# YikangZhang1641/merging-gym

Measured on AMD Instinct MI355X. Metric: env-steps/sec at batch=2^20; achieved HBM GB/s vs peak; 1/2/4/8-GPU scaling, higher is better.
Workload: dtype f64

## Files before the change

### merging-gym_amd/csrc/mg_qnet.h

```cpp
#pragma once

#include "mg_common.h"

namespace {

typedef __bf16 bf16x8 __attribute__((ext_vector_type(8)));
typedef float f32x16 __attribute__((ext_vector_type(16)));
typedef short i16x2 __attribute__((ext_vector_type(2)));
typedef __bf16 bf16x2 __attribute__((ext_vector_type(2)));

constexpr int kQH1Real = 200, kQH2Real = 100;
constexpr int kQT1 = 7;
constexpr int kQT2 = 7;
constexpr int kQK3 = 4;
constexpr int kQBiasIn = 13;
constexpr int kQOne1 = 200;
constexpr int kQOne2 = 100;
constexpr int kQMaxIn = kQBiasIn;
constexpr int kLMaxOut = 8;
static_assert(32 * kQT1 >= kQOne1 + 3 && 32 * (kQT1 - 1) < kQH1Real && 16 * kQT2 >= kQOne2 + 3 &&
                  16 * (kQT2 - 1) < kQH2Real && 32 * kQK3 >= 16 * kQT2,
              "tile counts cover the hidden units and their 1.0 units, no tile is all padding");

struct QFrag {
  int kind, tile, kb;
};
constexpr int kQFrags = 1 + 6 * 8 + 11;
__host__ __device__ constexpr QFrag qfrag(int s) {
  if (s == 0) return QFrag{0, 0, 0};
  if (s < 49) {
    const int u = s - 1, kb = u / 8, v = u % 8;
    return v == 0 ? QFrag{0, kb + 1, 0} : QFrag{1, v - 1, kb};
  }
  const int u = s - 49;
  if (u == 10) return QFrag{2, 0, 3};
  return u % 3 == 0 && u > 0 ? QFrag{2, 0, u / 3 - 1} : QFrag{1, u - u / 3, kQT1 - 1};
}
__host__ __device__ constexpr int qfrag_off(int s) {
  if (s <= 49) return 1024 * s;
  const int u = s - 49;
  return 1024 * s - 512 * ((u > 3) + (u > 6) + (u > 9) + (u > 10));
}
constexpr int kQNetBytes = qfrag_off(kQFrags);
static_assert(kQNetBytes == 56 * 1024 + 4 * 512, "7 W1 + 49 W2 fragments of 1 KB, 4 W3 of 512 B");

__host__ __device__ constexpr int qnet_unit1(int kb, int g, int j) {
  return 32 * kb + (j & 3) + 8 * (j >> 2) + 16 * (g & 1) + 4 * (g >> 1);
}
__host__ __device__ constexpr int qnet_unit2(int kb, int g, int j) {
  return 32 * kb + 16 * (j >> 2) + 4 * g + (j & 3);
}

__device__ __forceinline__ uint32_t relu_pair(float x, float y) {
  i16x2 v = __builtin_bit_cast(i16x2, __builtin_convertvector(f32x2{x, y}, bf16x2));
  const i16x2 zero = {0, 0};
  v = __builtin_elementwise_max(v, zero);
  return __builtin_bit_cast(uint32_t, v);
}

__device__ __forceinline__ bf16x8 qnet_input(const float* row, bool swap, int h) {
  float v[kObs];
#pragma unroll
  for (int k = 0; k < kObs / 2; ++k) {
    const f32x2 t = reinterpret_cast<const f32x2*>(row)[k];
    v[2 * k] = t[0];
    v[2 * k + 1] = t[1];
  }
  uint32_t pr[kObs / 2];
#pragma unroll
  for (int k = 0; k < kObs / 2; ++k) {
    const int a = swap ? (2 * k + 5) % kObs : 2 * k, b = swap ? (2 * k + 6) % kObs : 2 * k + 1;
    pr[k] = __builtin_bit_cast(uint32_t, __builtin_convertvector(f32x2{v[a], v[b]}, bf16x2));
  }
  static_assert(kQBiasIn == 13 && kObs == 10, "bias slots 13..15 follow the 10 features");
  const u32x4 w = h ? u32x4{pr[4], 0u, 0x3F800000u, 0x3F803F80u} : u32x4{pr[0], pr[1], pr[2], pr[3]};
  return __builtin_bit_cast(bf16x8, w);
}

__device__ __forceinline__ bf16x8 qnet_input_wide(const float* row16, int h) {
  const f32x4 lo = reinterpret_cast<const f32x4*>(row16 + 8 * h)[0];
  const f32x4 hi = reinterpret_cast<const f32x4*>(row16 + 8 * h)[1];
  const u32x4 w = {__builtin_bit_cast(uint32_t, __builtin_convertvector(f32x2{lo[0], lo[1]}, bf16x2)),
                   __builtin_bit_cast(uint32_t, __builtin_convertvector(f32x2{lo[2], lo[3]}, bf16x2)),
                   __builtin_bit_cast(uint32_t, __builtin_convertvector(f32x2{hi[0], hi[1]}, bf16x2)),
                   __builtin_bit_cast(uint32_t, __builtin_convertvector(f32x2{hi[2], hi[3]}, bf16x2))};
  return __builtin_bit_cast(bf16x8, w);
}

__device__ __forceinline__ f32x16 mfma32(bf16x8 a, bf16x8 b, f32x16 c) {
  return __builtin_amdgcn_mfma_f32_32x32x16_bf16(a, b, c, 0, 0, 0);
}
__device__ __forceinline__ f32x4 mfma16(bf16x8 a, bf16x8 b, f32x4 c) {
  return __builtin_amdgcn_mfma_f32_16x16x32_bf16(a, b, c, 0, 0, 0);
}

__global__ void qnet_pack_kernel(const float* w1, const float* b1, const float* w2, const float* b2,
                                 const float* w3, const float* b3, int in_dim, int out_dim,
                                 uint8_t* packed) {
  const int e = blockIdx.x * blockDim.x + threadIdx.x;
  if (e >= kQFrags * 64 * 8) return;
  const int s = e >> 9, lane = (e >> 3) & 63, j = e & 7;
  const QFrag f = qfrag(s);
  auto part = [](float b, int p) {
    const float hi = static_cast<float>(static_cast<__bf16>(b));
    const float r = b - hi;
    const float mid = static_cast<float>(static_cast<__bf16>(r));
    return p == 0 ? hi : p == 1 ? mid : r - mid;
  };
  float v = 0.f;
  int off = qfrag_off(s) + 16 * lane;
  if (f.kind == 0) {
    const int m = 32 * f.tile + (lane & 31), k = 8 * (lane >> 5) + j;
    if (m < kQH1Real && k < in_dim) v = w1[m * in_dim + k];
    else if (m < kQH1Real && k >= kQBiasIn && k < kQBiasIn + 3) v = part(b1[m], k - kQBiasIn);
    else if (m >= kQOne1 && m < kQOne1 + 3 && k == kQBiasIn) v = 1.f;
  } else if (f.kind == 1) {
    const int m = 16 * f.tile + (lane & 15), u = qnet_unit1(f.kb, lane >> 4, j);
    if (m < kQH2Real && u < kQH1Real) v = w2[m * kQH1Real + u];
    else if (m < kQH2Real && u >= kQOne1 && u < kQOne1 + 3) v = part(b2[m], u - kQOne1);
    else if (m >= kQOne2 && m < kQOne2 + 3 && u == kQOne1) v = 1.f;
  } else {
    if ((lane & 15) >= 8) return;
    const int m = lane & 7, u = qnet_unit2(f.kb, lane >> 4, j);
    if (m < out_dim && u < kQH2Real) v = w3[m * kQH2Real + u];
    else if (m < out_dim && u >= kQOne2 && u < kQOne2 + 3) v = part(b3[m], u - kQOne2);
    off = qfrag_off(s) + 16 * (8 * (lane >> 4) + m);
  }
  reinterpret_cast<__bf16*>(packed + off)[j] = static_cast<__bf16>(v);
}

__device__ __forceinline__ int opaque_zero() {
  int z = 0;
  asm volatile("" : "+v"(z));
  return z;
}

__device__ __forceinline__ void qnet_to_lds(const uint8_t* net, uint8_t* lds) {
  const f32x4* src = reinterpret_cast<const f32x4*>(net);
  f32x4* dst = reinterpret_cast<f32x4*>(lds);
  for (int j = threadIdx.x; j < kQNetBytes / 16; j += blockDim.x) dst[j] = src[j];
}

struct QSrcLds {
  const uint8_t* net;
  int lo, lo3;
  __device__ __forceinline__ bf16x8 operator()(int s) const {
    return *reinterpret_cast<const bf16x8*>(net + qfrag_off(s) + (qfrag(s).kind == 2 ? lo3 : lo));
  }
};
struct QSrcGlobal {
  __amdgpu_buffer_rsrc_t rs;
  int lo, lo3;
  __device__ __forceinline__ bf16x8 operator()(int s) const {
    return __builtin_bit_cast(
        bf16x8, __builtin_amdgcn_raw_buffer_load_b128(rs, qfrag(s).kind == 2 ? lo3 : lo, qfrag_off(s), 0));
  }
};
__device__ __forceinline__ int qnet_lane_off() { return 16 * (threadIdx.x & 63); }
__device__ __forceinline__ int qnet_lane_off3() {
  const int lane = threadIdx.x & 63;
  return 16 * (8 * (lane >> 4) + (lane & 7));
}
__device__ __forceinline__ QSrcLds qnet_lds(const uint8_t* net) {
  return QSrcLds{net + opaque_zero(), qnet_lane_off(), qnet_lane_off3()};
}
__device__ __forceinline__ QSrcGlobal qnet_global(const uint8_t* net) {
  return QSrcGlobal{__builtin_amdgcn_make_buffer_rsrc(const_cast<uint8_t*>(net), static_cast<short>(0), kQNetBytes,
                                                      0x00020000),
                    qnet_lane_off(), qnet_lane_off3()};
}
constexpr int kQLdsAhead = 2;
constexpr int kQGlobalAhead = 3;

__device__ __forceinline__ void permlane16_swap(uint32_t& x, uint32_t& y) {
  const uint32_t a = x, b = y;
  const uint64_t sw = __builtin_bit_cast(uint64_t, __builtin_amdgcn_permlane16_swap(a, b, false, false));
  x = static_cast<uint32_t>(sw);
  y = static_cast<uint32_t>(sw >> 32);
}

__device__ __forceinline__ void qnet_gather_q(const f32x4 (&acc3)[4], float (&q)[8]) {
  float x0[4], y0[4], x1[4], y1[4];
#pragma unroll
  for (int i = 0; i < 4; ++i) {
    x0[i] = acc3[0][i];
    y0[i] = acc3[2][i];
    x1[i] = acc3[1][i];
    y1[i] = acc3[3][i];
  }
  asm volatile(
      "s_nop 7\n\ts_nop 7\n\t"
      "v_permlane32_swap_b32 %0, %4\n\tv_permlane32_swap_b32 %8, %12\n\t"
      "v_permlane32_swap_b32 %1, %5\n\tv_permlane32_swap_b32 %9, %13\n\t"
      "v_permlane32_swap_b32 %2, %6\n\tv_permlane32_swap_b32 %10, %14\n\t"
      "v_permlane32_swap_b32 %3, %7\n\tv_permlane32_swap_b32 %11, %15\n\t"
      "s_nop 1\n\t"
      "v_permlane16_swap_b32 %0, %8\n\tv_permlane16_swap_b32 %1, %9\n\t"
      "v_permlane16_swap_b32 %2, %10\n\tv_permlane16_swap_b32 %3, %11\n\t"
      "s_nop 1"
      : "+v"(x0[0]), "+v"(x0[1]), "+v"(x0[2]), "+v"(x0[3]), "+v"(y0[0]), "+v"(y0[1]), "+v"(y0[2]), "+v"(y0[3]),
        "+v"(x1[0]), "+v"(x1[1]), "+v"(x1[2]), "+v"(x1[3]), "+v"(y1[0]), "+v"(y1[1]), "+v"(y1[2]), "+v"(y1[3]));
#pragma unroll
  for (int i = 0; i < 4; ++i) {
    q[i] = x0[i];
    q[4 + i] = x1[i];
  }
}

template <int D, int NC = 4, class Src>
__device__ __forceinline__ void qnet_mlp(const Src& src, bf16x8 xb0, bf16x8 xb1, float (&q)[8]) {
  static_assert(NC >= 1 && NC <= 4, "1..4 column tiles");
  constexpr int nc = NC;
  static_assert(kQT1 == 7 && kQT2 == 7 && kQK3 == 4 && kQFrags == 60,
                "qfrag's consumption order assumes 7 k-blocks, 7 layer-2 row tiles and 4 layer-3 k-blocks");
  bf16x8 ring[D];
#pragma unroll
  for (int s = 0; s < D; ++s) ring[s] = src(s);
  auto take = [&](int s) __attribute__((always_inline)) {
    const bf16x8 f = ring[s % D];
    if (s + D < kQFrags) ring[s % D] = src(s + D);
    return f;
  };
  const f32x16 z16 = {};
  const f32x4 z4 = {};
  f32x16 c0, c1;
  constexpr bool hi = nc > 2;
  auto layer1 = [&](int s) __attribute__((always_inline)) {
    const bf16x8 a1 = take(s);
    c0 = mfma32(a1, xb0, z16);
    if (hi) c1 = mfma32(a1, xb1, z16);
  };
  auto relu_d = [&](int d) __attribute__((always_inline)) {
    const f32x16& c = d < 8 ? c0 : c1;
    const int b = 2 * (d & 7);
    return relu_pair(c[b], c[b + 1]);
  };
  uint32_t nx[16];
  auto swap_u = [&](int u) __attribute__((always_inline)) {
#pragma unroll
    for (int qd = 0; qd < 4; ++qd) permlane16_swap(nx[8 * u + qd], nx[8 * u + 4 + qd]);
  };
  auto operands = [&](bf16x8 (&hb)[4]) __attribute__((always_inline)) {
#pragma unroll
    for (int t = 0; t < 4; ++t) hb[t] = __builtin_bit_cast(bf16x8, u32x4{nx[4 * t], nx[4 * t + 1], nx[4 * t + 2], nx[4 * t + 3]});
  };
  layer1(0);
#pragma unroll
  for (int d = 0; d < 8; ++d) nx[d] = relu_d(d);
  if (hi) {
#pragma unroll
    for (int d = 8; d < 16; ++d) nx[d] = relu_d(d);
  }
  swap_u(0);
  if (hi) swap_u(1);
  bf16x8 hb[4];
  operands(hb);
  f32x4 acc2[kQT2][4];
  auto slot = [&](f32x4& acc, const bf16x8& a, const bf16x8& b, bool zero) __attribute__((always_inline)) {
    __builtin_amdgcn_sched_barrier(0);
    acc = mfma16(a, b, zero ? z4 : acc);
  };
  int s = 1;
#pragma unroll
  for (int kb = 0; kb < kQT1 - 1; ++kb) {
    layer1(s++);
#pragma unroll
    for (int t2 = 0; t2 < kQT2; ++t2) {
      const bf16x8 a2 = take(s++);
#pragma unroll
      for (int t = 0; t < 4; ++t) {
        if (t < nc) slot(acc2[t2][t], a2, hb[t], kb == 0);
        if (t2 >= 1 && t2 <= 4 && (t2 <= 2 || hi)) nx[4 * (t2 - 1) + t] = relu_d(4 * (t2 - 1) + t);
        if (t2 == 5) permlane16_swap(nx[t], nx[4 + t]);
        if (t2 == 6 && hi) permlane16_swap(nx[8 + t], nx[12 + t]);
      }
    }
    operands(hb);
  }
  f32x4 acc3[4] = {z4, z4, z4, z4};
  uint32_t b3[2][4][4];
  auto pairs3 = [&](int t2, int t) __attribute__((always_inline)) {
    const int buf = (t2 >> 1) & 1, d = 2 * (t2 & 1);
    b3[buf][t][d] = relu_pair(acc2[t2][t][0], acc2[t2][t][1]);
    b3[buf][t][d + 1] = relu_pair(acc2[t2][t][2], acc2[t2][t][3]);
  };
  auto layer2 = [&](int t2, int p) __attribute__((always_inline)) {
    const bf16x8 a2 = take(s++);
#pragma unroll
    for (int t = 0; t < 4; ++t) {
      if (t < nc) slot(acc2[t2][t], a2, hb[t], false);
      if (p >= 0 && t < nc) pairs3(p, t);
    }
  };
  auto layer3 = [&](int k3, int p) __attribute__((always_inline)) {
    const bf16x8 a3 = take(s++);
    const int buf = k3 & 1;
#pragma unroll
    for (int t = 0; t < 4; ++t) {
      if (2 * k3 + 1 >= kQT2) b3[buf][t][2] = b3[buf][t][3] = 0u;
      const bf16x8 b = __builtin_bit_cast(bf16x8, u32x4{b3[buf][t][0], b3[buf][t][1], b3[buf][t][2], b3[buf][t][3]});
      if (t < nc) slot(acc3[t], a3, b, k3 == 0);
      if (p >= 0 && t < nc) pairs3(p, t);
    }
  };
  static_assert(kQT2 == 7 && kQK3 == 4, "the tail below is written for 7 row tiles, 4 layer-3 k-blocks");
  layer2(0, -1);
  layer2(1, 0);
  layer2(2, 1);
  layer3(0, 2);
  layer2(3, -1);
  layer2(4, 3);
  layer3(1, 4);
  layer2(5, -1);
  layer2(6, 5);
  layer3(2, 6);
  layer3(3, -1);
  qnet_gather_q(acc3, q);
}

template <int D, class Src>
__device__ __forceinline__ void qnet_mlp_nc(const Src& src, bf16x8 xb0, bf16x8 xb1, float (&q)[8], int nc) {
  switch (nc) {
    case 1:
      qnet_mlp<4 * D, 1>(src, xb0, xb1, q);
      break;
    case 2:
      qnet_mlp<2 * D, 2>(src, xb0, xb1, q);
      break;
    case 3:
      qnet_mlp<D + D / 2, 3>(src, xb0, xb1, q);
      break;
    default:
      qnet_mlp<D, 4>(src, xb0, xb1, q);
  }
}

__device__ __forceinline__ void qnet_mlp_swp(const uint8_t* net, bf16x8 xb0, bf16x8 xb1, float (&q)[8]) {
  qnet_mlp<kQLdsAhead>(qnet_lds(net), xb0, xb1, q);
}
__device__ __forceinline__ void qnet_mlp_swp_nc(const uint8_t* net, bf16x8 xb0, bf16x8 xb1, float (&q)[8], int nc) {
  qnet_mlp_nc<kQLdsAhead>(qnet_lds(net), xb0, xb1, q, nc);
}

__device__ __forceinline__ void qnet_forward_swp(const uint8_t* net, const float* tile, int row0,
                                                 bool swap, float (&q)[8]) {
  const int lane = threadIdx.x & 63, r = lane & 31, h = lane >> 5;
  qnet_mlp_swp(net, qnet_input(tile + (row0 + r) * kObs, swap, h),
               qnet_input(tile + (row0 + 32 + r) * kObs, swap, h), q);
}

constexpr int kQ32H1 = 224, kQ32H2 = 128;
constexpr int kQ32S1 = 24, kQ32S2 = 232, kQ32S3 = 136;
constexpr int kQ32R1 = 204, kQ32R2 = 104, kQ32R3 = 9;
constexpr int kQ32OffW2 = kQ32R1 * kQ32S1 * 2;
constexpr int kQ32OffW3 = kQ32OffW2 + kQ32R2 * kQ32S2 * 2;
constexpr int kQ32NetBytes = kQ32OffW3 + kQ32R3 * kQ32S3 * 2;
static_assert(kQ32OffW2 % 16 == 0 && kQ32OffW3 % 16 == 0 && kQ32NetBytes % 16 == 0 && kQNetBytes % 16 == 0,
              "packed Q-net sections must stay 16-byte aligned");

__device__ __forceinline__ int q32row1(int m) { return m < kQ32R1 ? m : kQ32R1 - 1; }
__device__ __forceinline__ int q32row2(int m) { return m < kQ32R2 ? m : kQ32R2 - 1; }
__device__ __forceinline__ int q32row3(int m) { return m < kQ32R3 ? m : kQ32R3 - 1; }

__host__ __device__ constexpr int q32_krow(int kk) {
  return 8 * ((kk & 7) >> 2) + 4 * (kk >> 3) + (kk & 3);
}

__device__ __forceinline__ bf16x8 relu_bf16(const f32x16& c, int s) {
  const int b = 8 * s;
  return __builtin_bit_cast(bf16x8, u32x4{relu_pair(c[b], c[b + 1]), relu_pair(c[b + 2], c[b + 3]),
                                          relu_pair(c[b + 4], c[b + 5]), relu_pair(c[b + 6], c[b + 7])});
}

__global__ void qnet32_pack_kernel(const float* w1, const float* b1, const float* w2, const float* b2,
                                 const float* w3, const float* b3, int in_dim, int out_dim,
                                 uint8_t* packed) {
  int e = blockIdx.x * blockDim.x + threadIdx.x;
  __bf16* pw1 = reinterpret_cast<__bf16*>(packed);
  __bf16* pw2 = reinterpret_cast<__bf16*>(packed + kQ32OffW2);
  __bf16* pw3 = reinterpret_cast<__bf16*>(packed + kQ32OffW3);
  auto part = [](float b, int p) {
    const float hi = static_cast<float>(static_cast<__bf16>(b));
    const float r = b - hi;
    const float mid = static_cast<float>(static_cast<__bf16>(r));
    return p == 0 ? hi : p == 1 ? mid : r - mid;
  };
  if (e < kQ32R1 * kQ32S1) {
    const int m = e / kQ32S1, k = e % kQ32S1;
    float v = 0.f;
    if (m < kQH1Real && k < in_dim) v = w1[m * in_dim + k];
    else if (m < kQH1Real && k >= kQBiasIn && k < kQBiasIn + 3) v = part(b1[m], k - kQBiasIn);
    else if (m >= kQOne1 && m < kQOne1 + 3 && k == kQBiasIn) v = 1.f;
    pw1[e] = static_cast<__bf16>(v);
    return;
  }
  e -= kQ32R1 * kQ32S1;
  if (e < kQ32R2 * kQ32S2) {
    const int m = e / kQ32S2, c = e % kQ32S2;
    const int src = 16 * (c / 16) + q32_krow(c % 16);
    float v = 0.f;
    if (c < kQ32H1) {
      if (m < kQH2Real && src < kQH1Real) v = w2[m * kQH1Real + src];
      else if (m < kQH2Real && src >= kQOne1 && src < kQOne1 + 3) v = part(b2[m], src - kQOne1);
      else if (m >= kQOne2 && m < kQOne2 + 3 && src == kQOne1) v = 1.f;
    }
    pw2[e] = static_cast<__bf16>(v);
    return;
  }
  e -= kQ32R2 * kQ32S2;
  if (e < kQ32R3 * kQ32S3) {
    const int m = e / kQ32S3, c = e % kQ32S3;
    const int src = 16 * (c / 16) + q32_krow(c % 16);
    float v = 0.f;
    if (m < out_dim && c < kQ32H2) {
      if (src < kQH2Real) v = w3[m * kQH2Real + src];
      else if (src >= kQOne2 && src < kQOne2 + 3) v = part(b3[m], src - kQOne2);
    }
    pw3[e] = static_cast<__bf16>(v);
  }
}

__device__ __forceinline__ void qnet32_gather_q(const f32x16& acc3_0, const f32x16& acc3_1, int h,
                                              float (&q)[8]) {
  (void)h;
#pragma unroll
  for (int j = 0; j < 4; ++j) {
    const float a = acc3_0[j], b = acc3_1[j];
    const uint32_t x = __builtin_bit_cast(uint32_t, a), y = __builtin_bit_cast(uint32_t, b);
    const uint64_t sw = __builtin_bit_cast(uint64_t, __builtin_amdgcn_permlane32_swap(x, y, false, false));
    q[j] = __builtin_bit_cast(float, static_cast<uint32_t>(sw));
    q[4 + j] = __builtin_bit_cast(float, static_cast<uint32_t>(sw >> 32));
  }
}

__device__ __forceinline__ void qnet32_mlp(const uint8_t* net, bf16x8 xb0, bf16x8 xb1, float (&q)[8]) {
  const int lane = threadIdx.x & 63, r = lane & 31, h = lane >> 5;
  const int z = opaque_zero();
  const __bf16* W1 = reinterpret_cast<const __bf16*>(net) + z;
  const __bf16* W2 = reinterpret_cast<const __bf16*>(net + kQ32OffW2) + z;
  const __bf16* W3 = reinterpret_cast<const __bf16*>(net + kQ32OffW3) + z;
  f32x16 acc2a[4] = {}, acc2b[4] = {};
  const f32x16 zero = {};
  auto layer1 = [&](int mt, f32x16& c0, f32x16& c1) {
    const bf16x8 a1 = *reinterpret_cast<const bf16x8*>(W1 + q32row1(32 * mt + r) * kQ32S1 + 8 * h);
    c0 = mfma32(a1, xb0, zero);
    c1 = mfma32(a1, xb1, zero);
  };
  f32x16 c0, c1;
  layer1(0, c0, c1);
  bf16x8 hb[4] = {relu_bf16(c0, 0), relu_bf16(c0, 1), relu_bf16(c1, 0), relu_bf16(c1, 1)};
  auto w2frag = [&](int mt, int j) {
    return *reinterpret_cast<const bf16x8*>(W2 + q32row2(32 * (j >> 1) + r) * kQ32S2 + 16 * (2 * mt + (j & 1)) + 8 * h);
  };
  auto tile_step = [&](int mt, bool more, int nk) __attribute__((always_inline)) {
    bf16x8 a2n = w2frag(mt, 0);
    if (more) layer1(mt + 1, c0, c1);
    uint32_t nx[16];
#pragma unroll
    for (int j = 0; j < 8; ++j) {
      const int m2 = j >> 1, sk = j & 1;
      if (sk >= nk) continue;
      const bf16x8 a2 = a2n;
      const int jn = nk == 2 ? j + 1 : j + 2;
      if (jn < 8) a2n = w2frag(mt, jn);
      __builtin_amdgcn_sched_barrier(0);
      acc2a[m2] = mfma32(a2, hb[sk], acc2a[m2]);
      acc2b[m2] = mfma32(a2, hb[2 + sk], acc2b[m2]);
      if (more) {
#pragma unroll
        for (int pp = 2 * j; pp < 2 * j + 2; ++pp) {
          const int f = pp >> 2, b = 8 * (f & 1) + 2 * (pp & 3);
          const f32x16& c = f < 2 ? c0 : c1;
          nx[pp] = relu_pair(c[b], c[b + 1]);
        }
      }
    }
    if (more) {
#pragma unroll
      for (int f = 0; f < 4; ++f)
        hb[f] = __builtin_bit_cast(bf16x8, u32x4{nx[4 * f], nx[4 * f + 1], nx[4 * f + 2], nx[4 * f + 3]});
    }
  };
  constexpr int kLast = kQ32H1 / 32 - 1;
  static_assert(16 * (2 * kLast + 1) >= kQH1Real && 32 * kLast < kQH1Real,
                "only the last hidden tile's second k-block is padding");
#pragma unroll
  for (int mt = 0; mt < kLast; ++mt) tile_step(mt, true, 2);
  f32x16 acc3_0 = {}, acc3_1 = {};
  auto w3frag = [&](int kb) { return *reinterpret_cast<const bf16x8*>(W3 + q32row3(r) * kQ32S3 + 16 * kb + 8 * h); };
  constexpr int kK3 = (kQH2Real + 15) / 16;
  static_assert(kK3 == 7 && kQ32H2 / 32 == 4, "layer 3 k-blocks 2 m2, 2 m2 + 1 follow layer-2 row tile m2");
  bf16x8 a3n = w3frag(0);
  auto layer3 = [&](int m2) __attribute__((always_inline)) {
#pragma unroll
    for (int sk = 0; sk < 2; ++sk) {
      const int kb = 2 * m2 + sk;
      if (kb >= kK3) continue;
      const bf16x8 a3 = a3n;
      if (kb + 1 < kK3) a3n = w3frag(kb + 1);
      acc3_0 = mfma32(a3, relu_bf16(acc2a[m2], sk), acc3_0);
      acc3_1 = mfma32(a3, relu_bf16(acc2b[m2], sk), acc3_1);
    }
  };
  bf16x8 a2n = w2frag(kLast, 0);
#pragma unroll
  for (int m2 = 0; m2 < kQ32H2 / 32; ++m2) {
    const bf16x8 a2 = a2n;
    if (m2 + 1 < kQ32H2 / 32) a2n = w2frag(kLast, 2 * (m2 + 1));
    __builtin_amdgcn_sched_barrier(0);
    acc2a[m2] = mfma32(a2, hb[0], acc2a[m2]);
    acc2b[m2] = mfma32(a2, hb[2], acc2b[m2]);
    if (m2 > 0) layer3(m2 - 1);
  }
  layer3(kQ32H2 / 32 - 1);
  qnet32_gather_q(acc3_0, acc3_1, h, q);
}

__device__ __forceinline__ void qnet32_forward(const uint8_t* net32, const float* tile, int row0, bool swap,
                                               float (&q)[8]) {
  const int lane = threadIdx.x & 63, r = lane & 31, h = lane >> 5;
  qnet32_mlp(net32, qnet_input(tile + (row0 + r) * kObs, swap, h), qnet_input(tile + (row0 + 32 + r) * kObs, swap, h), q);
}

__global__ __launch_bounds__(64) void qnet_fragments_kernel(const uint8_t* packed, uint8_t* frags) {
  const int i = blockIdx.x * 64 + threadIdx.x;
  if (i < kQNetBytes / 16) reinterpret_cast<u32x4*>(frags)[i] = reinterpret_cast<const u32x4*>(packed)[i];
}

__global__ __launch_bounds__(kBlock) void qnet_forward_kernel(const uint8_t* net, const float* x,
                                                              int in_dim, int swap, float* qout,
                                                              int64_t n) {
  __shared__ __attribute__((aligned(16))) uint8_t lds_net[kQNetBytes];
  __shared__ __attribute__((aligned(16))) float tile[kBlock * 16];
  const int64_t base = static_cast<int64_t>(blockIdx.x) * kBlock;
  qnet_to_lds(net, lds_net);
  for (int j = threadIdx.x; j < kBlock * 16; j += kBlock) {
    const int64_t i = base + (j >> 4);
    const int k = j & 15;
    const int src = swap ? (k + kObs / 2) % kObs : k;
    tile[j] = (i < n && k < in_dim) ? x[i * in_dim + src]
              : (k >= kQBiasIn && k < kQBiasIn + 3) ? 1.f : 0.f;
  }
  __syncthreads();
  float q[8];
  {
    const int lane = threadIdx.x & 63, row0 = (threadIdx.x >> 6) * 64;
    qnet_mlp_swp(lds_net, qnet_input_wide(tile + (row0 + (lane & 31)) * 16, lane >> 5),
                 qnet_input_wide(tile + (row0 + 32 + (lane & 31)) * 16, lane >> 5), q);
  }
  const int64_t i = base + threadIdx.x;
  if (i < n) {
#pragma unroll
    for (int j = 0; j < 8; ++j) qout[i * 8 + j] = q[j];
  }
}

}
```

### merging-gym_amd/csrc/mg_rollout_hdqn.h

```cpp
#pragma once

#include "mg_common.h"
#include "mg_env.h"
#include "mg_qnet.h"
#include "mg_rollout_qnet.h"
#include "mg_stats.h"
#include "mg_wave_out.h"

namespace {

__global__ void counter_add_kernel(uint64_t* counter, uint64_t k) { *counter += k; }

struct HRollout {
  mg_params P;
  Reset0 R0;
  mg_state S;
  mg_traj T;
  mg_hdqn_traj H;
  mg_stats St;
  int8_t* goal;
  int8_t* goal_op;
  double* ext_acc;
  const uint8_t* meta;
  const uint8_t* lower;
  const uint8_t* meta_op;
  const uint8_t* lower_op;
  uint64_t seed;
  uint64_t first_step;
  uint64_t greedy_thr;
  int64_t env_offset;
  int64_t n;
  int32_t num_steps;
  int32_t num_goals;
  int32_t reset_goal;
  uint32_t flags;
  float* ring;
  const uint64_t* ring_counter;
  int64_t ring_capacity;
};

constexpr int kHEnvs = 512;
constexpr int kRowGoalF = 2 * kObs + 4;
constexpr int kHHalf = kHEnvs / 2;
constexpr uint8_t kHGreedy = 0xFF;

__device__ __forceinline__ uint8_t draw_byte(uint32_t explore, uint32_t pick, uint64_t thr, int k) {
  return static_cast<uint8_t>(static_cast<uint64_t>(explore) < thr
                                  ? kHGreedy
                                  : (static_cast<uint64_t>(pick) * static_cast<uint64_t>(k)) >> 32);
}

template <int OPP>
__device__ __forceinline__ uint2 fresh_goal_words(uint64_t gi, uint64_t k, uint64_t seed, bool fresh, uint2& keep,
                                                  uint32_t& opp_word) {
  if constexpr (OPP == 1) {
    const uint4 u = philox_env_step(gi ^ (uint64_t{1} << 63), k, seed);
    opp_word = u.z;
    return make_uint2(u.x, u.y);
  } else {
    opp_word = 0u;
    if ((k & 1) == 0 || fresh) {
      const uint4 u = philox_env_step(gi ^ (uint64_t{1} << 63), k >> 1, seed);
      keep = make_uint2(u.z, u.w);
      return (k & 1) ? keep : make_uint2(u.x, u.y);
    }
    return keep;
  }
}

__device__ __forceinline__ bf16x8 qnet_input_goal(const float* row, int goal, int h, bool swap = false) {
  float v[kObs];
#pragma unroll
  for (int k = 0; k < kObs / 2; ++k) {
    const f32x2 t = reinterpret_cast<const f32x2*>(row)[k];
    const int d0 = swap ? (2 * k + kObs / 2) % kObs : 2 * k;
    const int d1 = swap ? (2 * k + 1 + kObs / 2) % kObs : 2 * k + 1;
    v[d0] = t[0];
    v[d1] = t[1];
  }
  auto pk = [](float a, float b) { return __builtin_bit_cast(uint32_t, __builtin_convertvector(f32x2{a, b}, bf16x2)); };
  const u32x4 w = h ? u32x4{pk(v[7], v[8]), pk(v[9], 0.f), 0x3F800000u, 0x3F803F80u}
                    : u32x4{pk(static_cast<float>(goal), v[0]), pk(v[1], v[2]), pk(v[3], v[4]), pk(v[5], v[6])};
  return __builtin_bit_cast(bf16x8, w);
}

__device__ __forceinline__ bf16x8 qnet_input_pairs(const uint32_t* side, int h) {
  return __builtin_bit_cast(bf16x8, h ? u32x4{side[4], 0u, 0x3F800000u, 0x3F803F80u}
                                      : u32x4{side[0], side[1], side[2], side[3]});
}

template <int OPP>
__global__ __launch_bounds__(512, 2) void hdqn_rollout_kernel(const HRollout R) {
  __shared__ __attribute__((aligned(16))) uint8_t lds_meta[kQNetBytes];
  __shared__ __attribute__((aligned(16))) uint8_t lds_lower[kQNetBytes];
  __shared__ __attribute__((aligned(16))) float tile[kHEnvs * kObs];
  __shared__ __attribute__((aligned(16))) uint32_t side[kHEnvs * 5];
  __shared__ uint8_t b_act[kHEnvs], b_goal[kHEnvs], b_done[kHEnvs], b_st_old[kHEnvs],
      b_st_new[kHEnvs], b_dg[kHEnvs], b_df[kHEnvs], b_g2[kHEnvs];
  constexpr bool kOpNets = OPP >= 2;
  __shared__ uint8_t b_aop[kOpNets ? kHEnvs : 1], b_gop[kOpNets ? kHEnvs : 1], b_dfo[kOpNets ? kHEnvs : 1];
  __shared__ uint8_t b_olist[kOpNets ? 4 : 1][64], b_gos[kOpNets ? kHEnvs : 1];

  const int tid = threadIdx.x, wave = tid >> 6, lane = tid & 63;
  const int64_t base = static_cast<int64_t>(blockIdx.x) * kHEnvs;
  const int T = R.num_steps;
  const int phases = 2 * T + 2;
  {
    const f32x4* s1 = reinterpret_cast<const f32x4*>(R.meta);
    const f32x4* s2 = reinterpret_cast<const f32x4*>(R.lower);
    f32x4* d1 = reinterpret_cast<f32x4*>(lds_meta);
    f32x4* d2 = reinterpret_cast<f32x4*>(lds_lower);
    for (int j = tid; j < kQNetBytes / 16; j += blockDim.x) {
      d1[j] = s1[j];
      d2[j] = s2[j];
    }
  }
  if (wave < 4) {
    __syncthreads();
    const int r = lane & 31, h = lane >> 5;
    for (int p = 0; p < phases; ++p) {
      const int g = p & 1, t = p >> 1;
      const int row0 = g * kHHalf + 64 * wave;
      const int j = row0 + lane;
      const int64_t i = base + j;
      const bool live = i < R.n;
      const int goal_prev = static_cast<int8_t>(b_goal[j]);
      const int dg = b_dg[j], df = b_df[j], st_new = b_st_new[j], st_old = b_st_old[j];
      const bool done = t > 0 && b_done[j] != 0;
      int gop_prev = 0, dfo = 0;
      if constexpr (kOpNets) {
        gop_prev = static_cast<int8_t>(b_gop[j]);
        dfo = b_dfo[j];
      }
      int goal_t;
      const bool need_meta = t > 0 || __ballot(live && goal_prev < 0) != 0;
      int gstar = 0;
      float qe = 0.f;
      if (need_meta) {
        const bool d0 = t > 0 && b_done[row0 + r], d1 = t > 0 && b_done[row0 + 32 + r];
        const bf16x8 p0 = qnet_input_pairs(side + (row0 + r) * 5, h), p1 = qnet_input_pairs(side + (row0 + 32 + r) * 5, h);
        const bf16x8 o0 = qnet_input(tile + (row0 + r) * kObs, false, h);
        const bf16x8 o1 = qnet_input(tile + (row0 + 32 + r) * kObs, false, h);
        const bf16x8 x0 = d0 ? p0 : o0, x1 = d1 ? p1 : o1;
        asm volatile("" ::"v"(dg), "v"(df), "v"(st_new), "v"(st_old), "v"(gop_prev), "v"(dfo));
        float q[8];
        qnet_mlp_swp(lds_meta, x0, x1, q);
        gstar = argmax_first(q, R.num_goals);
        const int g2 = dg == kHGreedy ? gstar : dg;
#pragma unroll
        for (int k = 0; k < 8; ++k) qe = k == g2 ? q[k] : qe;
      }
      bool brk = false;
      if (t > 0) {
        const int goal2 = dg == kHGreedy ? gstar : dg;
        brk = done || goal2 == st_new;
        goal_t = done ? (df == kHGreedy ? R.reset_goal : df) : (brk ? (df == kHGreedy ? gstar : df) : goal2);
        if (live) {
          const int64_t row = static_cast<int64_t>(t - 1) * R.n + i;
          if (R.H.next_goal) st_out(R.H.next_goal + row, static_cast<float>(goal2));
          if (R.H.reward) st_out(R.H.reward + row, goal2 == st_old ? 1.0f : 0.0f);
        }
        b_g2[j] = static_cast<uint8_t>(goal2);
        if (done && live) add_q_eval_nowait(R.St, i, static_cast<double>(qe));
      } else {
        goal_t = goal_prev >= 0 ? goal_prev : (df == kHGreedy ? gstar : df);
      }
      int gop_t = 0;
      if constexpr (kOpNets) {
        const bool fresh_op = t > 0 ? brk : gop_prev < 0;
        const bool need_o = live && fresh_op && dfo == kHGreedy;
        const uint64_t mo = __ballot(need_o);
        int gop_star = 0;
        if (mo != 0) {
          const int L = __popcll(mo);
          uint8_t* list = b_olist[wave];
          if (need_o) list[lane_rank(mo)] = static_cast<uint8_t>(lane);
          wave_lds_sync();
          const int ea = list[r < L ? r : 0], ec = list[32 + r < L ? 32 + r : 0], eo = list[lane < L ? lane : 0];
          float q[8];
          const bf16x8 x0 = qnet_input(tile + (row0 + ea) * kObs, true, h);
          const bf16x8 x1 = qnet_input(tile + (row0 + ec) * kObs, true, h);
          if constexpr (OPP == 3) {
            if (L <= 32)
              qnet_mlp<2 * kQGlobalAhead, 2>(qnet_global(R.meta_op), x0, x1, q);
            else
              qnet_mlp<kQGlobalAhead>(qnet_global(R.meta_op), x0, x1, q);
          } else {
            if (L <= 32)
              qnet_mlp<2 * kQLdsAhead, 2>(qnet_lds(lds_meta), x0, x1, q);
            else
              qnet_mlp_swp(lds_meta, x0, x1, q);
          }
          if (lane < L) b_gos[row0 + eo] = static_cast<uint8_t>(argmax_first(q, R.num_goals));
          wave_lds_sync();
          gop_star = b_gos[j];
        }
        gop_t = fresh_op ? (dfo == kHGreedy ? gop_star : dfo) : gop_prev;
      }
      if (t < T) {
        b_goal[j] = static_cast<uint8_t>(goal_t);
        if (live && R.H.goal) st_out(R.H.goal + static_cast<int64_t>(t) * R.n + i, static_cast<float>(goal_t));
        if constexpr (kOpNets) {
          b_gop[j] = static_cast<uint8_t>(gop_t);
          if (live && R.H.goal_op) st_out(R.H.goal_op + static_cast<int64_t>(t) * R.n + i, static_cast<float>(gop_t));
        }
        wave_lds_sync();
        const bf16x8 xe0 = qnet_input_goal(tile + (row0 + r) * kObs, b_goal[row0 + r], h);
        const bf16x8 xe1 = qnet_input_goal(tile + (row0 + 32 + r) * kObs, b_goal[row0 + 32 + r], h);
        bf16x8 xo0 = xe0, xo1 = xe1;
        if constexpr (kOpNets) {
          xo0 = qnet_input_goal(tile + (row0 + r) * kObs, b_gop[row0 + r], h, true);
          xo1 = qnet_input_goal(tile + (row0 + 32 + r) * kObs, b_gop[row0 + 32 + r], h, true);
        }
        float q[8];
        qnet_mlp_swp(lds_lower, xe0, xe1, q);
        b_act[j] = static_cast<uint8_t>(argmax_first(q, MG_NUM_ACTIONS));
        if constexpr (kOpNets) {
          float qo[8];
          const bf16x8 x0 = xo0, x1 = xo1;
          if constexpr (OPP == 3)
            qnet_mlp<kQGlobalAhead>(qnet_global(R.lower_op), x0, x1, qo);
          else
            qnet_mlp_swp(lds_lower, x0, x1, qo);
          b_aop[j] = static_cast<uint8_t>(argmax_first(qo, MG_NUM_ACTIONS));
        }
      } else if (live) {
        R.goal[i] = static_cast<int8_t>(goal_t);
        if constexpr (kOpNets) R.goal_op[i] = static_cast<int8_t>(gop_t);
      }
      __syncthreads();
    }
    return;
  }
  const int ew = wave - 4;
  Env e[2];
  bool live[2];
  double pend[2] = {0.0, 0.0};
  int stc[2];
  float ps[2][kObs], ps2[2][kObs];
  int pgoal[2], pact[2];
  const bool outer = R.ext_acc != nullptr;
  double acc[2] = {0.0, 0.0};
  uint2 kb[2] = {make_uint2(0u, 0u), make_uint2(0u, 0u)};
  auto finish_outer = [&](int g, int t, double& ac) __attribute__((always_inline)) {
    const int j = g * kHHalf + 64 * ew + lane;
    const int64_t i = base + j;
    const int64_t wbase = base + g * kHHalf + 64 * ew;
    const bool lv = i < R.n;
    const bool brk = b_done[j] != 0 || b_g2[j] == b_st_new[j];
    if (R.H.ext_reward && lv) st_out(R.H.ext_reward + static_cast<int64_t>(t) * R.n + i, static_cast<float>(ac));
    if (R.H.no_break) {
      const uint64_t m = __ballot(lv && !brk);
      if (lane == 0 && wbase < R.n) st_out(R.H.no_break + static_cast<int64_t>(t) * ((R.n + 63) >> 6) + (wbase >> 6), m);
    }
    if (brk) ac = 0.0;
  };
  const bool ring = R.ring != nullptr;
  const uint64_t c0 = ring ? *R.ring_counter : 0;
  const int64_t total = static_cast<int64_t>(T) * R.n;
  auto write_row = [&](int g, int t, const float (&s0)[kObs], const float (&s1)[kObs], int pg,
                       int pa) __attribute__((always_inline)) {
    const int j = g * kHHalf + 64 * ew + lane;
    const int64_t i = base + j;
    const int64_t k = static_cast<int64_t>(t) * R.n + i;
    if (!ring || i >= R.n || k < total - R.ring_capacity) return;
    const int goal2 = b_g2[j];
    const int st_old = b_st_old[j];
    float* row = R.ring + static_cast<int64_t>((c0 + static_cast<uint64_t>(k)) %
                                               static_cast<uint64_t>(R.ring_capacity)) * kRowGoalF;
    f32x4 v[6];
    float f[kRowGoalF];
    f[0] = static_cast<float>(pg);
#pragma unroll
    for (int q = 0; q < kObs; ++q) f[1 + q] = s0[q];
    f[11] = static_cast<float>(pa);
    f[12] = goal2 == st_old ? 1.0f : 0.0f;
    f[13] = static_cast<float>(goal2);
#pragma unroll
    for (int q = 0; q < kObs; ++q) f[14 + q] = s1[q];
#pragma unroll
    for (int q = 0; q < 6; ++q) v[q] = f32x4{f[4 * q], f[4 * q + 1], f[4 * q + 2], f[4 * q + 3]};
#pragma unroll
    for (int q = 0; q < 6; ++q) st_out(reinterpret_cast<f32x4*>(row) + q, v[q]);
  };
#pragma unroll
  for (int g = 0; g < 2; ++g) {
    const int j = g * kHHalf + 64 * ew + lane;
    const int64_t i = base + j;
    live[g] = i < R.n;
    double o[kObs];
    if (live[g]) {
      e[g] = load_env(R.S, i);
      pend[g] = pend_load(R.St, i, e[g]);
      double x1, y1, x2, y2;
      lon2coord(R.P, e[g].p1, true, x1, y1);
      lon2coord(R.P, e[g].p2, false, x2, y2);
      observe(R.P, e[g].p1, e[g].v1, e[g].p2, e[g].v2, x1, y1, x2, y2, o);
    } else {
      e[g].p1 = e[g].p2 = R.P.start_point;
      e[g].v1 = e[g].v2 = R.P.start_vel;
      e[g].ret1 = e[g].ret2 = 0.0;
      e[g].steps = 0;
      e[g].winner = 0;
      e[g].done = false;
#pragma unroll
      for (int k = 0; k < kObs; ++k) o[k] = 0.0;
    }
    stc[g] = goal_status(o[0], o[9]);
    float2* t2 = reinterpret_cast<float2*>(tile + j * kObs);
#pragma unroll
    for (int k = 0; k < kObs / 2; ++k) t2[k] = make_float2(static_cast<float>(o[2 * k]), static_cast<float>(o[2 * k + 1]));
    const uint64_t gi = static_cast<uint64_t>(R.env_offset + i);
    uint2 unused_keep;
    uint32_t unused_word;
    const uint2 fb = fresh_goal_words<OPP>(gi, R.first_step - 1, R.seed, true, unused_keep, unused_word);
    b_df[j] = draw_byte(fb.x, fb.y, R.greedy_thr, R.num_goals);
    b_goal[j] = live[g] ? static_cast<uint8_t>(R.goal[i]) : 0;
    if (outer && live[g]) acc[g] = R.ext_acc[i];
    if constexpr (kOpNets) {
      const uint4 fc = philox_env_step(gi ^ (uint64_t{1} << 62), R.first_step - 1, R.seed);
      b_dfo[j] = draw_byte(fc.z, fc.w, R.greedy_thr, R.num_goals);
      b_gop[j] = live[g] ? static_cast<uint8_t>(R.goal_op[i]) : 0;
    }
    b_done[j] = 0;
  }
  __syncthreads();
  for (int p = 0; p < phases; ++p) {
    if (p > 0 && ((p - 1) >> 1) < T) {
      const int g = (p - 1) & 1, t = (p - 1) >> 1;
      const int j = g * kHHalf + 64 * ew + lane;
      const int64_t i = base + j;
      const int64_t wbase = base + g * kHHalf + 64 * ew;
      const uint64_t gi = static_cast<uint64_t>(R.env_offset + i), k = R.first_step + t;
      const uint4 ua = philox_env_step(gi, k, R.seed);
      uint32_t opp_word;
      const uint2 ub = g == 0 ? fresh_goal_words<OPP>(gi, k, R.seed, t == 0, kb[0], opp_word)
                              : fresh_goal_words<OPP>(gi, k, R.seed, t == 0, kb[1], opp_word);
      const int a1 = static_cast<uint64_t>(ua.x) < R.greedy_thr ? static_cast<int>(b_act[j]) : action_from_u32(ua.y);
      int a2 = OPP == 1 ? action_from_u32(opp_word) : MG_ACTION_NONE;
      uint4 uc = make_uint4(0u, 0u, 0u, 0u);
      if constexpr (kOpNets) {
        uc = philox_env_step(gi ^ (uint64_t{1} << 62), k, R.seed);
        a2 = static_cast<uint64_t>(uc.x) < R.greedy_thr ? static_cast<int>(b_aop[j]) : action_from_u32(uc.y);
      }
      if (t > 0) {
        if (g == 0)
          write_row(0, t - 1, ps[0], ps2[0], pgoal[0], pact[0]);
        else
          write_row(1, t - 1, ps[1], ps2[1], pgoal[1], pact[1]);
        if (outer) {
          if (g == 0)
            finish_outer(0, t - 1, acc[0]);
          else
            finish_outer(1, t - 1, acc[1]);
        }
      }
      auto step = [&](Env& ev, bool lv, float (&s0)[kObs], float (&s1)[kObs], int& pg, int& pa, double& ac,
                      int& st, double& pd) __attribute__((always_inline)) {
        StepOut rv;
        b_st_old[j] = static_cast<uint8_t>(st);
        if (ring) {
          const f32x2* trow = reinterpret_cast<const f32x2*>(tile + j * kObs);
#pragma unroll
          for (int q = 0; q < kObs / 2; ++q) {
            const f32x2 v = trow[q];
            s0[2 * q] = v[0];
            s0[2 * q + 1] = v[1];
          }
          pg = b_goal[j];
          pa = a1;
        }
        env_step<false>(R.P, ev, a1, a2, rv);
        ac += rv.r1;
        if (ring) {
#pragma unroll
          for (int q = 0; q < kObs; ++q) s1[q] = static_cast<float>(rv.o[q]);
        }
        const int64_t row = static_cast<int64_t>(t) * R.n + i;
        if (lv) {
          if (R.T.rew) st_out(reinterpret_cast<f32x2*>(R.T.rew) + row, f32x2{static_cast<float>(rv.r1), static_cast<float>(rv.r2)});
          store_step_bytes(R.T, row, a1, a2, rv.done, rv.coll);
        }
        b_done[j] = rv.done ? 1 : 0;
        st = goal_status(rv.dx1, ev.v2);
        b_st_new[j] = static_cast<uint8_t>(st);
        b_dg[j] = draw_byte(ua.z, ua.w, R.greedy_thr, R.num_goals);
        b_df[j] = draw_byte(ub.x, ub.y, R.greedy_thr, R.num_goals);
        if constexpr (kOpNets) b_dfo[j] = draw_byte(uc.z, uc.w, R.greedy_thr, R.num_goals);
        const bool won = lv && ev.winner == 1;
        const int64_t rem = R.n - wbase;
        store_won_mask(R.T.won_mask, won, t, R.n, wbase, rem <= 0 ? 0 : (rem < 64 ? static_cast<int>(rem) : 64));
        if (lv && (R.flags & MG_AUTORESET) && rv.done) {
          uint32_t* sd = side + j * 5;
#pragma unroll
          for (int q2 = 0; q2 < kObs / 2; ++q2)
            sd[q2] = __builtin_bit_cast(uint32_t, __builtin_convertvector(
                                                      f32x2{static_cast<float>(rv.o[2 * q2]), static_cast<float>(rv.o[2 * q2 + 1])}, bf16x2));
          after_step_nowait(R.P, ev, rv, R.St, R.T.final_obs ? R.T.final_obs + row * kObs : nullptr, i, true, pd,
                            &R.R0);
          st = goal_status(rv.dx1, ev.v2);
        } else if (lv) {
          after_step_nowait(R.P, ev, rv, R.St, nullptr, i, false, pd, &R.R0);
        }
        const int64_t wrem = R.n - wbase;
        wave_store_obs(tile + (g * kHHalf + 64 * ew) * kObs, rv.o,
                       R.T.obs ? R.T.obs + (static_cast<int64_t>(t) * R.n + wbase) * kObs : nullptr,
                       wrem <= 0 ? 0 : (wrem < 64 ? static_cast<int>(wrem) : 64));
      };
      if (g == 0)
        step(e[0], live[0], ps[0], ps2[0], pgoal[0], pact[0], acc[0], stc[0], pend[0]);
      else
        step(e[1], live[1], ps[1], ps2[1], pgoal[1], pact[1], acc[1], stc[1], pend[1]);
    }
    __syncthreads();
  }
  write_row(0, T - 1, ps[0], ps2[0], pgoal[0], pact[0]);
  write_row(1, T - 1, ps[1], ps2[1], pgoal[1], pact[1]);
  if (outer) {
    finish_outer(0, T - 1, acc[0]);
    finish_outer(1, T - 1, acc[1]);
#pragma unroll
    for (int g = 0; g < 2; ++g)
      if (live[g]) R.ext_acc[base + g * kHHalf + 64 * ew + lane] = acc[g];
  }
#pragma unroll
  for (int g = 0; g < 2; ++g)
    if (live[g]) store_env(R.S, base + g * kHHalf + 64 * ew + lane, e[g]);
}

}
```

Baseline: 41.21 billion.

## Prefetch Q-net weight rings and env rows early in HDQN agent waves

Splits qnet_mlp into a prime step and a primed MLP so the weight-fragment ring for the meta and lower nets is loaded from LDS ahead of use, including across phase boundaries before the barrier. Env observation and side rows are loaded once into registers and reused for the meta and lower input builds. Goal values for the paired columns now come from a permlane swap instead of an LDS round trip, which removes a wave_lds_sync. It also specialises argmax and Q lookup for three goals. The cost is more live registers and scheduling barriers, which may add register pressure or spills.

Result: no change. 41.22 billion (median of 3 runs) (+0.0%).

```diff
diff --git a/merging-gym_amd/csrc/mg_qnet.h b/merging-gym_amd/csrc/mg_qnet.h
--- a/merging-gym_amd/csrc/mg_qnet.h
+++ b/merging-gym_amd/csrc/mg_qnet.h
@@ -207,15 +207,19 @@
   }
 }
 
+template <int D, class Src>
+__device__ __forceinline__ void qnet_prime(const Src& src, bf16x8 (&ring)[D]) {
+#pragma unroll
+  for (int s = 0; s < D; ++s) ring[s] = src(s);
+}
+
 template <int D, int NC = 4, class Src>
-__device__ __forceinline__ void qnet_mlp(const Src& src, bf16x8 xb0, bf16x8 xb1, float (&q)[8]) {
+__device__ __forceinline__ void qnet_mlp_primed(const Src& src, bf16x8 (&ring)[D], bf16x8 xb0, bf16x8 xb1,
+                                                float (&q)[8]) {
   static_assert(NC >= 1 && NC <= 4, "1..4 column tiles");
   constexpr int nc = NC;
   static_assert(kQT1 == 7 && kQT2 == 7 && kQK3 == 4 && kQFrags == 60,
                 "qfrag's consumption order assumes 7 k-blocks, 7 layer-2 row tiles and 4 layer-3 k-blocks");
-  bf16x8 ring[D];
-#pragma unroll
-  for (int s = 0; s < D; ++s) ring[s] = src(s);
   auto take = [&](int s) __attribute__((always_inline)) {
     const bf16x8 f = ring[s % D];
     if (s + D < kQFrags) ring[s % D] = src(s + D);
@@ -316,6 +320,13 @@
   layer3(2, 6);
   layer3(3, -1);
   qnet_gather_q(acc3, q);
+}
+
+template <int D, int NC = 4, class Src>
+__device__ __forceinline__ void qnet_mlp(const Src& src, bf16x8 xb0, bf16x8 xb1, float (&q)[8]) {
+  bf16x8 ring[D];
+  qnet_prime<D>(src, ring);
+  qnet_mlp_primed<D, NC>(src, ring, xb0, xb1, q);
 }
 
 template <int D, class Src>
diff --git a/merging-gym_amd/csrc/mg_rollout_hdqn.h b/merging-gym_amd/csrc/mg_rollout_hdqn.h
--- a/merging-gym_amd/csrc/mg_rollout_hdqn.h
+++ b/merging-gym_amd/csrc/mg_rollout_hdqn.h
@@ -68,25 +68,107 @@
   }
 }
 
-__device__ __forceinline__ bf16x8 qnet_input_goal(const float* row, int goal, int h, bool swap = false) {
+struct HRow {
+  f32x2 o[kObs / 2];
+  uint32_t s[kObs / 2];
+};
+__device__ __forceinline__ void hrow_load(const float* tile_row, const uint32_t* side_row, HRow& w) {
+#pragma unroll
+  for (int k = 0; k < kObs / 2; ++k) {
+    w.o[k] = reinterpret_cast<const f32x2*>(tile_row)[k];
+    w.s[k] = side_row[k];
+  }
+}
+__device__ __forceinline__ void hrow_pin(HRow& a, HRow& b) {
+  asm volatile("" : "+v"(a.o[0]), "+v"(a.o[1]), "+v"(a.o[2]), "+v"(a.o[3]), "+v"(a.o[4]), "+v"(b.o[0]), "+v"(b.o[1]),
+               "+v"(b.o[2]), "+v"(b.o[3]), "+v"(b.o[4]));
+  asm volatile("" : "+v"(a.s[0]), "+v"(a.s[1]), "+v"(a.s[2]), "+v"(a.s[3]), "+v"(a.s[4]), "+v"(b.s[0]), "+v"(b.s[1]),
+               "+v"(b.s[2]), "+v"(b.s[3]), "+v"(b.s[4]));
+}
+
+__device__ __forceinline__ void hrow_load_tile(const float* tile_row, HRow& w) {
+#pragma unroll
+  for (int k = 0; k < kObs / 2; ++k) w.o[k] = reinterpret_cast<const f32x2*>(tile_row)[k];
+}
+__device__ __forceinline__ void hrow_pin_tile(HRow& a, HRow& b) {
+  asm volatile("" : "+v"(a.o[0]), "+v"(a.o[1]), "+v"(a.o[2]), "+v"(a.o[3]), "+v"(a.o[4]), "+v"(b.o[0]), "+v"(b.o[1]),
+               "+v"(b.o[2]), "+v"(b.o[3]), "+v"(b.o[4]));
+}
+
+__device__ __forceinline__ uint32_t pk_bf16(float a, float b) {
+  return __builtin_bit_cast(uint32_t, __builtin_convertvector(f32x2{a, b}, bf16x2));
+}
+
+__device__ __forceinline__ bf16x8 hrow_meta_input(const HRow& w, bool ended, int h) {
+  uint32_t m[kObs / 2];
+#pragma unroll
+  for (int k = 0; k < kObs / 2; ++k) m[k] = ended ? w.s[k] : pk_bf16(w.o[k][0], w.o[k][1]);
+  return __builtin_bit_cast(bf16x8, h ? u32x4{m[4], 0u, 0x3F800000u, 0x3F803F80u} : u32x4{m[0], m[1], m[2], m[3]});
+}
+
+__device__ __forceinline__ bf16x8 hrow_input(const HRow& w, bool swap, int h) {
   float v[kObs];
 #pragma unroll
   for (int k = 0; k < kObs / 2; ++k) {
-    const f32x2 t = reinterpret_cast<const f32x2*>(row)[k];
+    v[2 * k] = w.o[k][0];
+    v[2 * k + 1] = w.o[k][1];
+  }
+  uint32_t pr[kObs / 2];
+#pragma unroll
+  for (int k = 0; k < kObs / 2; ++k) {
+    const int a = swap ? (2 * k + 5) % kObs : 2 * k, b = swap ? (2 * k + 6) % kObs : 2 * k + 1;
+    pr[k] = pk_bf16(v[a], v[b]);
+  }
+  return __builtin_bit_cast(bf16x8, h ? u32x4{pr[4], 0u, 0x3F800000u, 0x3F803F80u} : u32x4{pr[0], pr[1], pr[2], pr[3]});
+}
+
+__device__ __forceinline__ bf16x8 hrow_goal_input(const HRow& w, int goal, int h, bool swap = false) {
+  float v[kObs];
+#pragma unroll
+  for (int k = 0; k < kObs / 2; ++k) {
     const int d0 = swap ? (2 * k + kObs / 2) % kObs : 2 * k;
     const int d1 = swap ? (2 * k + 1 + kObs / 2) % kObs : 2 * k + 1;
-    v[d0] = t[0];
-    v[d1] = t[1];
-  }
-  auto pk = [](float a, float b) { return __builtin_bit_cast(uint32_t, __builtin_convertvector(f32x2{a, b}, bf16x2)); };
-  const u32x4 w = h ? u32x4{pk(v[7], v[8]), pk(v[9], 0.f), 0x3F800000u, 0x3F803F80u}
-                    : u32x4{pk(static_cast<float>(goal), v[0]), pk(v[1], v[2]), pk(v[3], v[4]), pk(v[5], v[6])};
-  return __builtin_bit_cast(bf16x8, w);
-}
-
-__device__ __forceinline__ bf16x8 qnet_input_pairs(const uint32_t* side, int h) {
-  return __builtin_bit_cast(bf16x8, h ? u32x4{side[4], 0u, 0x3F800000u, 0x3F803F80u}
-                                      : u32x4{side[0], side[1], side[2], side[3]});
+    v[d0] = w.o[k][0];
+    v[d1] = w.o[k][1];
+  }
+  const float g = static_cast<float>(goal);
+  const u32x4 x = {pk_bf16(h ? v[7] : g, h ? v[8] : v[0]), pk_bf16(h ? v[9] : v[1], h ? 0.f : v[2]),
+                   h ? 0x3F800000u : pk_bf16(v[3], v[4]), h ? 0x3F803F80u : pk_bf16(v[5], v[6])};
+  return __builtin_bit_cast(bf16x8, x);
+}
+
+__device__ __forceinline__ int argmax_goals(const float (&q)[8], int num_goals) {
+  int best;
+  if (num_goals == 3) {
+    const bool b1 = q[1] > q[0];
+    const float v = b1 ? q[1] : q[0];
+    best = q[2] > v ? 2 : (b1 ? 1 : 0);
+    asm volatile("" : "+v"(best));
+  } else {
+    best = argmax_first(q, num_goals);
+    asm volatile("" : "+v"(best));
+  }
+  return best;
+}
+__device__ __forceinline__ float q_of_goal(const float (&q)[8], int g, int num_goals) {
+  float qe = 0.f;
+  if (num_goals == 3) {
+#pragma unroll
+    for (int k = 0; k < 3; ++k) qe = k == g ? q[k] : qe;
+    asm volatile("" : "+v"(qe));
+  } else {
+#pragma unroll
+    for (int k = 0; k < 8; ++k) qe = k == g ? q[k] : qe;
+    asm volatile("" : "+v"(qe));
+  }
+  return qe;
+}
+
+__device__ __forceinline__ void column_values(int x, int& lo, int& hi) {
+  const uint32_t a = static_cast<uint32_t>(x), b = a;
+  const uint64_t sw = __builtin_bit_cast(uint64_t, __builtin_amdgcn_permlane32_swap(a, b, false, false));
+  lo = static_cast<int>(static_cast<uint32_t>(sw));
+  hi = static_cast<int>(static_cast<uint32_t>(sw >> 32));
 }
 
 template <int OPP>
@@ -118,38 +200,57 @@
   if (wave < 4) {
     __syncthreads();
     const int r = lane & 31, h = lane >> 5;
+    bf16x8 ring_meta[kQLdsAhead];
+    constexpr bool kPrimeAhead = !kOpNets;
+    if constexpr (kPrimeAhead) qnet_prime(qnet_lds(lds_meta), ring_meta);
     for (int p = 0; p < phases; ++p) {
       const int g = p & 1, t = p >> 1;
       const int row0 = g * kHHalf + 64 * wave;
       const int j = row0 + lane;
       const int64_t i = base + j;
       const bool live = i < R.n;
-      const int goal_prev = static_cast<int8_t>(b_goal[j]);
-      const int dg = b_dg[j], df = b_df[j], st_new = b_st_new[j], st_old = b_st_old[j];
-      const bool done = t > 0 && b_done[j] != 0;
-      int gop_prev = 0, dfo = 0;
+      if constexpr (!kPrimeAhead) qnet_prime(qnet_lds(lds_meta), ring_meta);
+      uint32_t by_goal = b_goal[j], by_dg = b_dg[j], by_df = b_df[j], by_new = b_st_new[j], by_old = b_st_old[j];
+      uint32_t by_done = b_done[j], by_d0 = b_done[row0 + r], by_d1 = b_done[row0 + 32 + r];
+      uint32_t by_gop = 0, by_dfo = 0;
       if constexpr (kOpNets) {
-        gop_prev = static_cast<int8_t>(b_gop[j]);
-        dfo = b_dfo[j];
-      }
+        by_gop = b_gop[j];
+        by_dfo = b_dfo[j];
+      }
+      HRow w0, w1;
+      hrow_load(tile + (row0 + r) * kObs, side + (row0 + r) * 5, w0);
+      hrow_load(tile + (row0 + 32 + r) * kObs, side + (row0 + 32 + r) * 5, w1);
+      asm volatile("" : "+v"(by_goal), "+v"(by_dg), "+v"(by_df), "+v"(by_new), "+v"(by_old), "+v"(by_done), "+v"(by_d0),
+                   "+v"(by_d1), "+v"(by_gop), "+v"(by_dfo));
+      hrow_pin(w0, w1);
+      uint32_t held0 = by_dg | by_df << 8 | by_new << 16 | by_old << 24;
+      uint32_t held1 = by_goal | by_done << 8 | by_gop << 16 | by_dfo << 24;
+      asm volatile("" : "+v"(held0), "+v"(held1));
+      const int dg = held0 & 0xFF, df = held0 >> 8 & 0xFF, st_new = held0 >> 16 & 0xFF, st_old = held0 >> 24;
+      const int goal_prev = static_cast<int8_t>(held1);
+      const bool done = (held1 >> 8 & 0xFF) != 0;
+      const int gop_prev = static_cast<int8_t>(held1 >> 16), dfo = held1 >> 24;
       int goal_t;
       const bool need_meta = t > 0 || __ballot(live && goal_prev < 0) != 0;
       int gstar = 0;
       float qe = 0.f;
       if (need_meta) {
-        const bool d0 = t > 0 && b_done[row0 + r], d1 = t > 0 && b_done[row0 + 32 + r];
-        const bf16x8 p0 = qnet_input_pairs(side + (row0 + r) * 5, h), p1 = qnet_input_pairs(side + (row0 + 32 + r) * 5, h);
-        const bf16x8 o0 = qnet_input(tile + (row0 + r) * kObs, false, h);
-        const bf16x8 o1 = qnet_input(tile + (row0 + 32 + r) * kObs, false, h);
-        const bf16x8 x0 = d0 ? p0 : o0, x1 = d1 ? p1 : o1;
-        asm volatile("" ::"v"(dg), "v"(df), "v"(st_new), "v"(st_old), "v"(gop_prev), "v"(dfo));
+        const bf16x8 x0 = hrow_meta_input(w0, by_d0 != 0, h), x1 = hrow_meta_input(w1, by_d1 != 0, h);
         float q[8];
-        qnet_mlp_swp(lds_meta, x0, x1, q);
-        gstar = argmax_first(q, R.num_goals);
-        const int g2 = dg == kHGreedy ? gstar : dg;
-#pragma unroll
-        for (int k = 0; k < 8; ++k) qe = k == g2 ? q[k] : qe;
-      }
+        qnet_mlp_primed<kQLdsAhead>(qnet_lds(lds_meta), ring_meta, x0, x1, q);
+        gstar = argmax_goals(q, R.num_goals);
+        qe = q_of_goal(q, dg == kHGreedy ? gstar : dg, R.num_goals);
+      }
+      const QSrcLds src_lower = qnet_lds(lds_lower);
+      bf16x8 ring_lower[kQLdsAhead];
+      HRow l0, l1;
+      auto lower_reads = [&]() __attribute__((always_inline)) {
+        qnet_prime(src_lower, ring_lower);
+        const float* rows = tile + opaque_zero();
+        hrow_load_tile(rows + (row0 + r) * kObs, l0);
+        hrow_load_tile(rows + (row0 + 32 + r) * kObs, l1);
+      };
+      if constexpr (!kOpNets) lower_reads();
       bool brk = false;
       if (t > 0) {
         const int goal2 = dg == kHGreedy ? gstar : dg;
@@ -176,10 +277,14 @@
           uint8_t* list = b_olist[wave];
           if (need_o) list[lane_rank(mo)] = static_cast<uint8_t>(lane);
           wave_lds_sync();
-          const int ea = list[r < L ? r : 0], ec = list[32 + r < L ? 32 + r : 0], eo = list[lane < L ? lane : 0];
+          int ea = list[r < L ? r : 0], ec = list[32 + r < L ? 32 + r : 0], eo = list[lane < L ? lane : 0];
+          asm volatile("" : "+v"(ea), "+v"(ec), "+v"(eo));
           float q[8];
-          const bf16x8 x0 = qnet_input(tile + (row0 + ea) * kObs, true, h);
-          const bf16x8 x1 = qnet_input(tile + (row0 + ec) * kObs, true, h);
+          HRow wa, wc;
+          hrow_load_tile(tile + (row0 + ea) * kObs, wa);
+          hrow_load_tile(tile + (row0 + ec) * kObs, wc);
+          hrow_pin_tile(wa, wc);
+          const bf16x8 x0 = hrow_input(wa, true, h), x1 = hrow_input(wc, true, h);
           if constexpr (OPP == 3) {
             if (L <= 32)
               qnet_mlp<2 * kQGlobalAhead, 2>(qnet_global(R.meta_op), x0, x1, q);
@@ -191,29 +296,34 @@
             else
               qnet_mlp_swp(lds_meta, x0, x1, q);
           }
-          if (lane < L) b_gos[row0 + eo] = static_cast<uint8_t>(argmax_first(q, R.num_goals));
+          if (lane < L)
+            b_gos[row0 + eo] = static_cast<uint8_t>(OPP == 3 ? argmax_first(q, R.num_goals) : argmax_goals(q, R.num_goals));
           wave_lds_sync();
           gop_star = b_gos[j];
         }
         gop_t = fresh_op ? (dfo == kHGreedy ? gop_star : dfo) : gop_prev;
+        lower_reads();
       }
       if (t < T) {
         b_goal[j] = static_cast<uint8_t>(goal_t);
+        int ge0, ge1;
+        column_values(goal_t & 0xFF, ge0, ge1);
+        hrow_pin_tile(l0, l1);
+        const bf16x8 xe0 = hrow_goal_input(l0, ge0, h), xe1 = hrow_goal_input(l1, ge1, h);
+        bf16x8 xo0 = xe0, xo1 = xe1;
+        if constexpr (kOpNets) {
+          b_gop[j] = static_cast<uint8_t>(gop_t);
+          int go0, go1;
+          column_values(gop_t & 0xFF, go0, go1);
+          xo0 = hrow_goal_input(l0, go0, h, true);
+          xo1 = hrow_goal_input(l1, go1, h, true);
+        }
         if (live && R.H.goal) st_out(R.H.goal + static_cast<int64_t>(t) * R.n + i, static_cast<float>(goal_t));
         if constexpr (kOpNets) {
-          b_gop[j] = static_cast<uint8_t>(gop_t);
           if (live && R.H.goal_op) st_out(R.H.goal_op + static_cast<int64_t>(t) * R.n + i, static_cast<float>(gop_t));
         }
-        wave_lds_sync();
-        const bf16x8 xe0 = qnet_input_goal(tile + (row0 + r) * kObs, b_goal[row0 + r], h);
-        const bf16x8 xe1 = qnet_input_goal(tile + (row0 + 32 + r) * kObs, b_goal[row0 + 32 + r], h);
-        bf16x8 xo0 = xe0, xo1 = xe1;
-        if constexpr (kOpNets) {
-          xo0 = qnet_input_goal(tile + (row0 + r) * kObs, b_gop[row0 + r], h, true);
-          xo1 = qnet_input_goal(tile + (row0 + 32 + r) * kObs, b_gop[row0 + 32 + r], h, true);
-        }
         float q[8];
-        qnet_mlp_swp(lds_lower, xe0, xe1, q);
+        qnet_mlp_primed<kQLdsAhead>(src_lower, ring_lower, xe0, xe1, q);
         b_act[j] = static_cast<uint8_t>(argmax_first(q, MG_NUM_ACTIONS));
         if constexpr (kOpNets) {
           float qo[8];
@@ -227,6 +337,9 @@
       } else if (live) {
         R.goal[i] = static_cast<int8_t>(goal_t);
         if constexpr (kOpNets) R.goal_op[i] = static_cast<int8_t>(gop_t);
+      }
+      if constexpr (kPrimeAhead) {
+        if (p + 1 < phases) qnet_prime(qnet_lds(lds_meta), ring_meta);
       }
       __syncthreads();
     }
```
